# OllieBoyne/sslap

Hardware: AMD Instinct MI355X
Metric: Medges/s (bid-phase CSR nnz/s) + solve ms, N=200k d=0.1% sparse LAP (higher is better)
Workload: dtype f64

## Files before the change

### sslap_amd/csrc/host_base.hpp

```cpp
#pragma once

namespace {

thread_local std::string g_err;

int fail(int code, const char *fmt, ...) {
    char buf[512];
    va_list ap;
    va_start(ap, fmt);
    vsnprintf(buf, sizeof(buf), fmt, ap);
    va_end(ap);
    g_err = buf;
    return code;
}

#define HIP_TRY(expr)                                                                              \
    do {                                                                                           \
        hipError_t _e = (expr);                                                                    \
        if (_e != hipSuccess)                                                                      \
            return fail(MISSLAP_ERR_HIP, "%s failed: %s (%s:%d)", #expr, hipGetErrorString(_e), __FILE__, \
                        __LINE__);                                                                 \
    } while (0)

double now_ms() {
// ... 72 lines not shown
int block_alloc(void **p, size_t bytes, size_t *got);
void block_free(int device, void *p, size_t bytes);
}

namespace {
struct BatchFiber;
}
struct misslap_solver {
    BatchFiber *batch = nullptr;
    int abi = MISSLAP_ABI_VERSION;
    int n_cus = 256;
    double lines_safe_eps = 0.0;
    bool lines_dropped = false;
    double max_abs = 0.0;
    double pmax0 = 0.0;
    float eps_start_opt = 0.f;
    bool untouched = true;
    bool dense = false;
    int64_t dense_cols = 0;
    int device = 0;
    hipStream_t stream = nullptr;
    bool own_stream = false;
    int64_t nnz = 0;
    int n_rows = 0, n_cols = 0;
    int maximize = 0;
    bool f32 = true;
    int2 *edges32 = nullptr;
    int *col = nullptr;
    double *val64 = nullptr;
    int *row_ptr = nullptr;
    double *price = nullptr;
    float *price32 = nullptr;
    int *pmax_bits = nullptr;
    float cmax32 = 0.f;
    float *price32_buf = nullptr;
    PriceRec *rec = nullptr;
    int2 *cand = nullptr;
    double *cand64 = nullptr;
    int *p2o = nullptr, *o2p = nullptr, *U = nullptr;
    unsigned long long *bid_key = nullptr;
    int *bid_obj = nullptr;
    int4 *bid_rec = nullptr;
    unsigned long long *best_key = nullptr;
    int *best_pos = nullptr;
    int *cnt = nullptr, *hole_list = nullptr, *mover_list = nullptr;
    int *need_list = nullptr;
    Ctl *ctl = nullptr;
    double *contrib = nullptr;
    int *nmatch = nullptr;
    FinSlot *fin_slots = nullptr;
    int fin_slots_n = 0;
    unsigned long long *launch_edges = nullptr;
    int launch_edges_cap = 0;
    unsigned *tiled = nullptr;
    int tiled_fmt = 0;
    int *seg4 = nullptr;
    int *tcol = nullptr;
    int *ovf_ptr = nullptr;
    int4 *ovf_q = nullptr;
    int ovf_cap = 0;
    double2 *part_vw = nullptr;
    int *part_g = nullptr;
    unsigned long long *wg_stats = nullptr;
    int wg_stats_slots = 0;
    int take_edges_n = 0;
    unsigned long long *take_edges_out = nullptr;
    int *split_cnt = nullptr;
    int n_tiled = 0;
    int tile_cols = 0;
    long long tile_L = 0;
    int T = 0;
    bool tiled_ok = false;
    int tiled_min_K = 0;
    int tiled_shape = 0;
    std::vector<Blk> blocks;
    Ctl *h_ctl = nullptr;
    Ctl *h_stat = nullptr;
    volatile unsigned long long *live = nullptr;
    unsigned long long *live_dev = nullptr;
    unsigned ticket = 0;
    bool live_valid = false;
    bool live_off = false;
    bool live_every_round = false;
    unsigned slot_ticket[2] = {0, 0};
    bool slot_live[2] = {false, false};
    hipEvent_t stat_ev[2] = {nullptr, nullptr};
    float eps = 0, target_eps = 0, theta = 0, start_eps = 0;
    int nreductions = 0;
    bool finished = false;
    int64_t max_iter = 0;
    int thr = -1;
    bool round_small = false;
    bool round_fused = true;
    bool round_done = false;
    int cand_build_max_K = 0x7fffffff;
    int tail_round_budget = kLongRowTailBudget;
    int tail_launch_rounds = 1 << 22;
    int max_row_len = 0;
    long long avg_row_len = 0;
    bool lines_live() const { return cand != nullptr && !lines_dropped && (avg_row_len <= kCandRowMax || long_rows); }
    bool long_rows_later = false;
    long long tail_rounds_host = 0;
    long long tail_nits0 = -1;
    bool long_rows = false;
    bool long_rows0 = false, long_rows_later0 = false;
    bool line_maintenance = true;
    int cand_refresh_min = kDefaultCandRefresh;
    bool round_ordered = false;
    int apply_bidders_ratio = 2;
    bool profile_all = false;
    int rounds_per_sync = kDefaultRoundsPerSync;
    bool rounds_per_sync_auto = true;
    int rank = 0, world = 1;
    long long sharded_rounds = 0;
    int phases_run = 0, phases_with_lines = 0;
    int shard_min_K = 0;
    bool profile = false;
    int K_ub = 0;
    bool K_exact = false;
    bool walk_rev_next = false;
    bool ece_flag_clear = false;
    int ctl_fresh = 0;
    bool phase_fresh = true;
    std::vector<ProfRec> prof;
    size_t prof_used = 0;
    int launch_idx = 0;
    double setup_ms = 0, solve_ms = 0;
};
```

### sslap_amd/csrc/host_rounds.hpp

```cpp
#pragma once

namespace {
void begin_phase(misslap_solver *h) {
    if (h->cand != nullptr && !h->lines_dropped && (double)h->eps < h->lines_safe_eps) h->lines_dropped = true;
    h->phases_run += 1;
    h->phases_with_lines += h->lines_live() ? 1 : 0;
}

RoundArgs round_args(misslap_solver *h) {
    RoundArgs a;
    a.ctl = h->ctl;
    a.row_ptr = h->row_ptr;
    a.price = h->price;
    a.rec = h->rec;
    a.p2o = h->p2o;
    a.o2p = h->o2p;
    a.U = h->U;
    a.bid_key = h->bid_key;
    a.bid_obj = h->bid_obj;
    a.bid_rec = h->bid_rec;
    a.best_key = h->best_key;
    a.best_pos = h->best_pos;
    a.cnt = h->cnt;
    a.hole_list = h->hole_list;
// ... 17 lines not shown
    a.cand_build_max_K = h->cand_build_max_K;
    a.cand_build_min_K = (h->thr > 0 && h->line_maintenance) ? kRoundSmallMax : 0;
    a.cand_refresh_min = h->cand_refresh_min;
    a.price32 = nullptr;
    a.pmax_bits = h->pmax_bits;
    a.cmax = h->cmax32;
    return a;
}

int blocks_for(long long items, int per_block) {
    long long b = (items + per_block - 1) / per_block;
    if (b < 1) b = 1;
    if (b > kMaxGridBlocks) b = kMaxGridBlocks;
    return (int)b;
}

ProfRec *prof_next(misslap_solver *h, int kind) {
    if (h->prof_used == h->prof.size()) {
        ProfRec r{};
        if (hipEventCreate(&r.start) != hipSuccess || hipEventCreate(&r.stop) != hipSuccess) return nullptr;
        h->prof.push_back(r);
    }
    ProfRec *r = &h->prof[h->prof_used++];
    r->kind = kind;
    r->fullscan = 0;
    r->launch_idx = -1;
    return r;
}

void count_tail_rounds(misslap_solver *h) {
    if (h->tail_nits0 < 0) return;
    h->tail_rounds_host += h->h_ctl->nits - h->tail_nits0;
    h->tail_nits0 = -1;
}

int read_ctl(misslap_solver *h) {
    if (h->ctl_fresh == 2) {
        if (h->h_ctl->err)
            return fail(MISSLAP_ERR_STATE, "device-side invariant violated (error bits 0x%x)", h->h_ctl->err);
        return MISSLAP_OK;
    }
    HIP_TRY(stream_memcpy(h, h->h_ctl, h->ctl, sizeof(Ctl), hipMemcpyDeviceToHost));
    HIP_TRY(stream_sync(h));
    h->ctl_fresh = 2;
    h->K_ub = h->h_ctl->K;
    h->K_exact = true;
    count_tail_rounds(h);
    if (h->h_ctl->err)
        return fail(MISSLAP_ERR_STATE, "device-side invariant violated (error bits 0x%x)", h->h_ctl->err);
    return MISSLAP_OK;
}

bool live_poll(misslap_solver *h, unsigned want, bool exact, int *K, int *err, long long *nits) {
    volatile unsigned long long *w = h->live;
    double t_end = now_ms() + 20000.0;
    for (unsigned spins = 0;; ++spins) {
        const unsigned long long a = w[0], b = w[1], c = w[2], d = w[3];
        const unsigned t = (unsigned)(a >> 32);
        if ((unsigned)(b >> 32) == t && (unsigned)(c >> 32) == t && (unsigned)(d >> 32) == t && w[0] == a &&
            (exact ? t == want : (int)(t - want) >= 0)) {
            *K = (int)(unsigned)(a & 0xffffffffull);
            *err = (int)(unsigned)(b & 0xffffffffull);
            *nits = (long long)((c & 0xffffffffull) | ((d & 0xffffffffull) << 32));
            return true;
        }
        if (h->batch) {
            batch_yield(h, BatchFiber::kPolling);
            if (h->batch->at < h->batch->pending.size()) t_end = now_ms() + 20000.0;
            else if ((spins & 255) == 255 && now_ms() > t_end) return false;
        } else if (spins < 4000) {
            __builtin_ia32_pause();
        } else {
            std::this_thread::yield();
            if ((spins & 1023) == 0 && now_ms() > t_end) return false;
        }
    }
}
void ensure_posted(misslap_solver *h) {
    if (h->live_valid || h->live_off) return;
    launch<k_post_status>(h, dim3(1), h->ctl, h->live_dev, ++h->ticket);
    h->live_valid = true;
}
int read_status(misslap_solver *h) {
    if (h->ctl_fresh == 2 || h->live_off) return read_ctl(h);
    if (h->ctl_fresh == 1) {
        if (h->h_ctl->err) return fail(MISSLAP_ERR_STATE, "device-side invariant violated (error bits 0x%x)", h->h_ctl->err);
        return MISSLAP_OK;
    }
    ensure_posted(h);
    int K = 0, err = 0;
    long long nits = 0;
    if (!live_poll(h, h->ticket, true, &K, &err, &nits)) {
        h->live_off = true;
        return read_ctl(h);
    }
    h->h_ctl->K = K;
    h->h_ctl->nits = nits;
    h->h_ctl->err = err;
    h->K_ub = K;
    h->K_exact = true;
    count_tail_rounds(h);
    if (err) return fail(MISSLAP_ERR_STATE, "device-side invariant violated (error bits 0x%x)", err);
    return MISSLAP_OK;
}

int status_enqueue(misslap_solver *h, int slot) {
    h->slot_live[slot] = !h->live_off;
    if (h->slot_live[slot]) {
        ensure_posted(h);
        h->slot_ticket[slot] = h->ticket;
        return MISSLAP_OK;
    }
    h->ctl_fresh = false;
    if (h->batch) return fail(MISSLAP_ERR_STATE, "a batched solve needs the live status words");
    HIP_TRY(hipMemcpyAsync(&h->h_stat[slot], h->ctl, sizeof(Ctl), hipMemcpyDeviceToHost, h->stream));
    HIP_TRY(hipEventRecord(h->stat_ev[slot], h->stream));
    return MISSLAP_OK;
}
int status_wait(misslap_solver *h, int slot) {
    if (h->slot_live[slot]) {
        int K = 0, err = 0;
        long long nits = 0;
        if (live_poll(h, h->slot_ticket[slot], false, &K, &err, &nits)) {
            h->h_stat[slot].K = K;
            h->h_stat[slot].nits = nits;
            h->h_stat[slot].err = err;
            h->K_ub = K;
            h->K_exact = false;
            if (err) return fail(MISSLAP_ERR_STATE, "device-side invariant violated (error bits 0x%x)", err);
            return MISSLAP_OK;
        }
        h->live_off = true;
        int rc = read_ctl(h);
        h->h_stat[slot] = *h->h_ctl;
        h->K_exact = false;
        return rc;
    }
    HIP_TRY(hipEventSynchronize(h->stat_ev[slot]));
    const Ctl &c = h->h_stat[slot];
    h->K_ub = c.K;
    h->K_exact = false;
    if (c.err) return fail(MISSLAP_ERR_STATE, "device-side invariant violated (error bits 0x%x)", c.err);
    return MISSLAP_OK;
}

bool walk_backwards(misslap_solver *h, const int *shp) {
    const bool can = MISSLAP_TILED_KEYCOL_ON && h->tiled_fmt <= 1 && shp[7] == 1 &&
                     (h->tiled_shape == 0 || h->tiled_shape == 8 || h->tiled_shape == 9);
    if (h->phase_fresh) h->walk_rev_next = false;
    const bool rev = can && h->walk_rev_next;
    h->walk_rev_next = !h->walk_rev_next;
    return rev;
}

int launch_bid_tiled(misslap_solver *h) {
    h->ctl_fresh = false;
    RoundArgs a = round_args(h);
    const bool sharded = h->world > 1 && h->K_exact && h->K_ub >= h->shard_min_K;
    const long long share = sharded ? ((long long)h->K_ub + h->world - 1) / h->world : h->K_ub;
    const int *shp = kTiledShapes[h->tiled_shape];
    const int groups = (shp[0] - 64 * shp[5]) / shp[6];
    const int per_wg_max = groups * shp[1];
    const int cs = shp[7];
    long long grid = (share + per_wg_max - 1) / per_wg_max;
    const long long resident = h->n_cus / cs;
    const long long spread = std::min<long long>(resident, (share + groups - 1) / groups);
    if (grid < spread) grid = spread;
    grid *= cs;
    TiledArgs ta{h->tiled, h->tcol, h->seg4, h->T, h->tiled_min_K, h->n_tiled,
                 nullptr, nullptr, h->ovf_ptr, h->ovf_q, h->ovf_cap, h->part_vw, h->part_g, h->n_rows, h->split_cnt, FinalOut{}};
    h->round_ordered = !h->phase_fresh;
    if (h->round_ordered) {
        int *pos_of = h->nmatch, *order_person = h->hole_list, *order_pos = h->mover_list, *sums = h->cnt;
        const int nchunks = (h->n_rows + kScanChunk - 1) / kScanChunk;
        launch<k_order_prepare>(h, dim3(std::max(nchunks, blocks_for(h->K_ub, k_order_prepare::kBlock))), h->ctl, h->U, pos_of, h->p2o,
                                h->n_rows, nchunks, sums, h->thr, h->tiled_min_K);
        launch<k_order_scatter>(h, dim3(nchunks), h->ctl, h->p2o, h->n_rows, sums, pos_of, order_person, order_pos, h->thr, h->tiled_min_K);
        ta.order_person = order_person;
        ta.order_pos = order_pos;
    }
    if (grid > h->wg_stats_slots) return fail(MISSLAP_ERR_STATE, "scan grid %lld exceeds the statistics slots (%d)", grid, h->wg_stats_slots);
    ProfRec *pr = nullptr;
    if (h->profile) {
        if (h->launch_idx >= h->launch_edges_cap)
            return fail(MISSLAP_ERR_STATE, "profile buffer exhausted (%d bid launches)", h->launch_idx);
        pr = prof_next(h, 2);
        if (!pr) return fail(MISSLAP_ERR_HIP, "hipEventCreate failed");
        pr->fullscan = h->phase_fresh;
        pr->launch_idx = a.launch_idx = h->launch_idx++;
    }
    const size_t lds = tiled_lds_bytes(shp[4]);
    const dim3 g((unsigned)grid);
    if (walk_backwards(h, shp)) {
        const int key = h->tiled_fmt * 100 + shp[6];
        switch (key) {
#define X(FMT, GL) \
    case FMT * 100 + GL: launch_alone(h, pr, MISSLAP_BID_KERNEL_REV(GL, FMT), g, dim3(1024), lds, a, ta); break;
            X(0, 4) X(0, 8) X(0, 16) X(1, 4) X(1, 8) X(1, 16)
#undef X
            default: return fail(MISSLAP_ERR_STATE, "no backward instance for format %d with %d lanes per person", h->tiled_fmt, shp[6]);
        }
    } else if (h->tiled_fmt == 0) {
        switch (h->tiled_shape) {
#define X(I, TH, R, B, D, TC, LD, GL, CS) \
    case I: launch_alone(h, pr, k_bid_tiled<TH, R, B, D, TC, LD, 0, GL, CS>, g, dim3(TH), lds, a, ta); break;
            MISSLAP_FOR_TILED_SHAPES(X)
#undef X
            default: return fail(MISSLAP_ERR_STATE, "bad tiled shape");
        }
    } else {
        const int key = h->tiled_fmt * 100 + shp[6];
        switch (key) {
#define X(FMT, GL) \
    case FMT * 100 + GL: launch_alone(h, pr, MISSLAP_BID_KERNEL_FMT(GL, FMT), g, dim3(1024), lds, a, ta); break;
            MISSLAP_FOR_FMT_LANES(X)
#undef X
            default: return fail(MISSLAP_ERR_STATE, "no full-scan instance for format %d with %d lanes per person", h->tiled_fmt, shp[6]);
        }
    }
    if (pr) {
        h->take_edges_n = (int)grid;
        h->take_edges_out = h->launch_edges + 2 * (size_t)pr->launch_idx;
    }
    HIP_TRY(hipGetLastError());
    return MISSLAP_OK;
}

bool use_round_small(const misslap_solver *h) {
    return h->K_ub <= kRoundSmallMax && (h->world == 1 || h->K_ub < h->shard_min_K);
}

int launch_bid(misslap_solver *h) {
    h->ctl_fresh = false;
    h->untouched = false;
    h->round_small = use_round_small(h) && !(h->tiled_ok && h->K_ub >= h->tiled_min_K);
    if (h->tiled_ok && h->K_ub >= h->tiled_min_K) {
        int rc = launch_bid_tiled(h);
        if (rc) return rc;
        if (h->K_exact) {
            h->phase_fresh = false;
            h->K_exact = false;
            return MISSLAP_OK;
        }
    }
    h->K_exact = false;
    RoundArgs a = round_args(h);
    const long long share = h->K_ub;
    const bool fused = h->round_small && h->round_fused;
    const int grid = blocks_for(share, (fused ? 1024 : kBidBlock) / kWave);
    ProfRec *pr = nullptr;
    const bool fullscan = h->phase_fresh && !(h->tiled_ok && h->K_ub >= h->tiled_min_K);
    if (!(h->profile && (h->profile_all || fullscan))) a.launch_edges = nullptr;
    if (h->profile && (h->profile_all || fullscan)) {
        if (h->launch_idx >= h->launch_edges_cap)
            return fail(MISSLAP_ERR_STATE, "profile buffer exhausted (%d bid launches)", h->launch_idx);
        pr = prof_next(h, 0);
        if (!pr) return fail(MISSLAP_ERR_HIP, "hipEventCreate failed");
        pr->fullscan = fullscan;
        pr->launch_idx = a.launch_idx = h->launch_idx++;
    }
    const EdgesF32 e32{h->edges32};
    const EdgesF64 e64{h->col, h->val64};
    const dim3 g(grid);
    if (fused) {
        a.live = (h->live_off || !h->live_every_round) ? nullptr : h->live_dev;
        a.ticket = ++h->ticket;
        h->live_valid = a.live != nullptr;
    }
    const int variant = !h->lines_live() ? 0 : h->K_ub > h->cand_build_max_K ? 1 : 2;
    if (h->price32 && !h->round_small && variant != 2 && (long long)h->K_ub * 8 >= h->n_rows) {
        HIP_TRY(stream_memset(h, h->pmax_bits, 0, sizeof(int)));
        launch<k_price_mirror>(h, dim3(std::min(blocks_for(h->n_cols, k_price_mirror::kBlock * 4), h->n_cus)), h->ctl, h->price, h->price32,
                               h->n_cols, h->pmax_bits, h->thr, a.gather_max_K);
        a.price32 = h->price32;
    }
    const auto bid = [&](auto ed) {
        using E = decltype(ed);
        if (fused) launch_timed<k_round_fused<E>>(h, pr, g, a, ed);
        else if (h->round_small) launch_timed<k_bid<E, RecSource, 2>>(h, pr, g, a, ed);
        else if (variant == 0) launch_timed<k_bid<E, PriceSource, 0>>(h, pr, g, a, ed);
        else if (variant == 1) launch_timed<k_bid<E, PriceSource, 1>>(h, pr, g, a, ed);
        else launch_timed<k_bid<E, PriceSource, 2>>(h, pr, g, a, ed);
    };
    if (h->f32) bid(e32);
    else bid(e64);
    if (pr && !h->round_small) {
        h->take_edges_n = std::max(h->take_edges_n, grid);
        h->take_edges_out = h->launch_edges + 2 * (size_t)pr->launch_idx;
    } else if (pr) {
        hipLaunchKernelGGL(k_take_launch_edges, dim3(1), dim3(1024), 0, h->stream, h->wg_stats, grid, h->launch_edges + 2 * (size_t)pr->launch_idx);
    }
    HIP_TRY(hipGetLastError());
    h->phase_fresh = false;
    h->round_done = fused;
    return MISSLAP_OK;
}

int launch_tiebreak(misslap_solver *h) {
    h->ctl_fresh = false;
    if (h->round_small) return MISSLAP_OK;
    RoundArgs a = round_args(h);
    const long long share = h->K_ub;
    launch<k_tiebreak>(h, dim3(blocks_for(share, k_tiebreak::kBlock)), a, h->round_ordered ? h->mover_list : nullptr, h->tiled_min_K,
                       h->take_edges_n, h->take_edges_out);
    h->take_edges_n = 0;
    h->take_edges_out = nullptr;
    HIP_TRY(hipGetLastError());
    return MISSLAP_OK;
}

int launch_apply(misslap_solver *h) {
    h->ctl_fresh = false;
    if (h->round_small && h->round_done) {
        h->round_small = h->round_done = false;
        h->K_exact = false;
        return MISSLAP_OK;
    }
    RoundArgs a = round_args(h);
    a.live = (h->live_off || (h->round_small && !h->live_every_round)) ? nullptr : h->live_dev;
    a.ticket = ++h->ticket;
    h->live_valid = a.live != nullptr;
    if (h->round_small) {
        h->round_small = false;
        h->K_exact = false;
        launch<k_round_small>(h, dim3(1), a);
        HIP_TRY(hipGetLastError());
        return MISSLAP_OK;
    }
    h->K_exact = false;
    h->round_ordered = false;
    if ((h->world == 1 || h->K_ub < h->shard_min_K) && (long long)h->K_ub * h->apply_bidders_ratio <= h->n_cols)
        launch<k_apply_bidders>(h, dim3(blocks_for(h->K_ub, k_apply_bidders::kBlock)), a);
    else
        launch<k_apply>(h, dim3(blocks_for(h->n_cols, k_apply::kBlock)), a);
    if (h->K_ub <= kCompactSmallMax) {
        launch<k_compact_small>(h, dim3(1), a);
    } else {
        const int cb = blocks_for(h->K_ub, kChunk);
        launch<k_compact_count>(h, dim3(cb), a);
        launch<k_compact_scatter>(h, dim3(cb), a);
        launch<k_compact_fill>(h, dim3(blocks_for(h->K_ub, k_compact_fill::kBlock)), a);
    }
    HIP_TRY(hipGetLastError());
    return MISSLAP_OK;
}

int launch_tail(misslap_solver *h) {
    if (h->thr <= 0) return MISSLAP_OK;
// ... 169 lines not shown
```

### sslap_amd/csrc/kernels_round.hpp

```cpp
#pragma once
#include "device_common.hpp"

namespace misslap {

struct RoundArgs {
    Ctl *ctl;
    const int *row_ptr;
    double *price;
    PriceRec *rec;
    int *p2o;
    int *o2p;
    int *U;
    unsigned long long *bid_key;
    int *bid_obj;
    int4 *bid_rec;
    unsigned long long *best_key;
    int *best_pos;
    int *cnt;
    int *hole_list;
    int *mover_list;
    unsigned long long *launch_edges;
    int n_rows, n_cols;
    int thr;
    int rank, world;
// ... 43 lines not shown

constexpr int kBidBlock = 256;
template <class Src>
struct SrcOf;
template <>
struct SrcOf<PriceSource> {
    static constexpr bool kOwners = false;
    static __device__ __forceinline__ PriceSource make(const RoundArgs &a) { return PriceSource{a.price}; }
};
template <>
struct SrcOf<RecSource> {
    static constexpr bool kOwners = true;
    static __device__ __forceinline__ RecSource make(const RoundArgs &a) { return RecSource{a.rec}; }
};
struct BidTally {
    unsigned long long edges = 0, hit_edges = 0;
    int nb = 0, nh = 0, err = 0;
};
__device__ __forceinline__ void handover_store(unsigned long long *p, unsigned long long v) {
    __hip_atomic_store(p, v, __ATOMIC_RELAXED, __HIP_MEMORY_SCOPE_AGENT);
}
__device__ __forceinline__ unsigned long long handover_load(const unsigned long long *p) {
    return __hip_atomic_load(p, __ATOMIC_RELAXED, __HIP_MEMORY_SCOPE_AGENT);
}

template <class E, class Src, int kLines, bool kHandOver>
__device__ __forceinline__ void bid_positions(const RoundArgs &a, const E &ed, int lo, int hi, int first, int stride,
                                              int i_first, BidTally &tl) {
    const int lane = threadIdx.x & 63;
    const double eps = (double)a.eps;
    const Src src = SrcOf<Src>::make(a);
    double hint = 0.0;
    const bool lines = kLines > 0 && E::kCand && a.cand != nullptr;
    for (int n = lo + first; n < hi; n += stride) {
        const int i = n == first ? i_first : a.U[n];
        const int s = a.row_ptr[i], e = a.row_ptr[i + 1];
        CandBid b[2];
        b[0].hit = false;
        if (lines) {
            typename E::Slot sl = LineIO<typename E::Slot>::load(a.cand, a.cand64,
                                                                 (size_t)i * kCandLanes + (lane & (kCandLanes - 1)));
            int alive[2];
            cand_eval2(sl, true, false, src, eps, b, tl.err, NoEarly(), NoStamp(), alive);
            if (kLines == 2 && alive[0] < a.cand_refresh_min) b[0].hit = false;
        }
        if (!b[0].hit) {
            if (kLines == 2) {
                CandBuildArgs ba;
                const typename E::Raw none[4] = {};
                wave_bid_full<E, Src, false, false>(ed, src, s, e, none, eps, b[0], ba, tl.err);
                if (lines && ba.want && hi > a.cand_build_min_K) cand_build(a.cand, a.cand64, i, ba, eps, hint);
            } else if (!SrcOf<Src>::kOwners && a.price32 != nullptr) {
                const float two_delta = 0x1p-21f * (a.cmax + __int_as_float(*a.pmax_bits));
                wave_bid_filter(ed, a.price, a.price32, two_delta, s, e, eps, b[0], tl.err);
            } else {
                wave_bid_lean(ed, src, s, e, eps, b[0], tl.err);
            }
        } else {
            tl.nh += 1;
            tl.hit_edges += (unsigned long long)b[0].len;
        }
        if (lane == 0) {
            if (kHandOver) {
                handover_store(&a.bid_key[n], b[0].key);
                unsigned long long *r = reinterpret_cast<unsigned long long *>(&a.bid_rec[n]);
                handover_store(r, (unsigned long long)(unsigned)b[0].obj | ((unsigned long long)(unsigned)b[0].prev << 32));
                handover_store(r + 1, (unsigned long long)(unsigned)i | ((unsigned long long)(unsigned)s << 32));
            } else {
                a.bid_key[n] = b[0].key;
                if (SrcOf<Src>::kOwners) {
                    a.bid_rec[n] = make_int4(b[0].obj, b[0].prev, i, s);
                } else {
                    a.bid_obj[n] = b[0].obj;
                    atomicMax(&a.best_key[b[0].obj], b[0].key);
                }
            }
        }
        tl.edges += (unsigned long long)b[0].len;
        tl.nb += 1;
    }
}

template <int kWaves>
__device__ __forceinline__ void tally_flush(const RoundArgs &a, const BidTally &tl, int K) {
    const int wave = threadIdx.x >> 6, lane = threadIdx.x & 63;
    __shared__ unsigned long long s_edges[kWaves], s_hedges[kWaves];
    __shared__ int s_nb[kWaves], s_nh[kWaves];
    if (lane == 0) {
        s_edges[wave] = tl.edges;
        s_hedges[wave] = tl.hit_edges;
        s_nb[wave] = tl.nb;
        s_nh[wave] = tl.nh;
        if (tl.err) atomicOr(&a.ctl->err, tl.err);
    }
    __syncthreads();
    if (threadIdx.x == 0) {
        unsigned long long te = 0, the = 0;
        int tb = 0, th = 0;
        for (int w = 0; w < kWaves; ++w) {
            te += s_edges[w];
            the += s_hedges[w];
            tb += s_nb[w];
            th += s_nh[w];
        }
        if (tb) {
            unsigned long long *st = a.wg_stats + (size_t)kStatWords * blockIdx.x;
            st[kStatEdges] += te;
            st[kStatBids] += (unsigned long long)tb;
            if (a.world > 1 && K >= a.shard_min_K) st[kStatShardEdges] += te;
            if (a.launch_edges) {
                st[kStatLaunchEdges] += te;
                st[kStatLaunchHitEdges] += the;
            }
            if (th) {
                st[kStatHits] += (unsigned long long)th;
                st[kStatHitEdges] += the;
            }
        }
    }
}

template <class E, class Src, int kLines>
struct k_bid {
    MISSLAP_KERNEL(kBidBlock)
    static __device__ __forceinline__ void run(RoundArgs a, E ed) {
        static_assert(kLines == 2 || !SrcOf<Src>::kOwners, "the lean scan does not carry the owners k_round_small needs");
        const int wave = threadIdx.x >> 6;
        const int wpb = kBidBlock / kWave;
        const int first = blockIdx.x * wpb + wave;
        const Ctl *ctl = a.ctl;
        const CtlHead head(ctl);
        const int i_first = a.U[min(first, a.n_rows - 1)];
        if (!head.live(a.thr, i_first < -1)) return;
        if (a.gather_max_K > 0 && head.K >= a.gather_max_K) return;
        int lo, hi;
        shard_range(head.K, a.rank, a.world, a.shard_min_K, lo, hi);
        BidTally tl;
        bid_positions<E, Src, kLines, false>(a, ed, lo, hi, first, gridDim.x * wpb, i_first, tl);
        tally_flush<kBidBlock / kWave>(a, tl, head.K);
    }
};


struct k_price_mirror {
    MISSLAP_KERNEL(1024)
    static __device__ __forceinline__ void run(const Ctl *ctl, const double *price, float *price32, int n_cols, int *pmax_bits, int thr, int gather_max_K) {
        if (!round_live(ctl, thr) || (gather_max_K > 0 && ctl->K >= gather_max_K)) return;
        __shared__ int s_w[16];
        float m = 0.f;
        for (int j = blockIdx.x * blockDim.x + threadIdx.x; j < n_cols; j += gridDim.x * blockDim.x) {
            const float p = (float)price[j];
            price32[j] = p;
            m = __builtin_fmaxf(m, __builtin_fabsf(p));
        }
        int b = __float_as_int(m);
        for (int off = 32; off >= 1; off >>= 1) b = max(b, __shfl_xor(b, off));
        if ((threadIdx.x & 63) == 0) s_w[threadIdx.x >> 6] = b;
        __syncthreads();
        if (threadIdx.x == 0) {
            for (int w = 1; w < (int)blockDim.x / kWave; ++w) b = max(b, s_w[w]);
            if (b > 0) atomicMax(pmax_bits, b);
        }
    }
};


template <class E>
struct k_refresh_lines {
    MISSLAP_KERNEL(kBidBlock)
    static __device__ __forceinline__ void run(RoundArgs a, E ed, int min_alive, int long_max, int min_alive_long) {
        if (!E::kCand || a.cand == nullptr) return;
        const int wave = threadIdx.x >> 6, lane = threadIdx.x & 63;
        const int wpb = kBidBlock / kWave;
        const double eps = (double)a.eps;
        const PriceSource src{a.price};
        double hint = 0.0;
        int err = 0;
        for (int w = blockIdx.x * wpb + wave; 2 * w < a.n_rows; w += gridDim.x * wpb) {
            const int i0 = 2 * w, i1 = 2 * w + 1;
            const bool act1 = i1 < a.n_rows;
            const int ime = (lane < kCandLanes || !act1) ? i0 : i1;
            typename E::Slot sl = LineIO<typename E::Slot>::load(a.cand, a.cand64,
                                                                 (size_t)ime * kCandLanes + (lane & (kCandLanes - 1)));
            CandBid b[2];
            int alive[2];
            cand_eval2(sl, true, act1, src, eps, b, err, NoEarly(), NoStamp(), alive);
#pragma unroll
            for (int X = 0; X < 2; ++X) {
                if (X == 1 && !act1) continue;
                if (b[X].hit && alive[X] >= max(min_alive, min_alive_long)) continue;
                const int i = X ? i1 : i0;
                const int s = a.row_ptr[i], e = a.row_ptr[i + 1];
                if (e - s > kCandRowMax) {
                    if (long_max > 0 && e - s <= long_max && !(b[X].hit && alive[X] >= min_alive_long) && lane == 0)
                        a.need_list[atomicAdd(&a.ctl->n_need, 1)] = i;
                    continue;
                }
                if (b[X].hit && alive[X] >= min_alive) continue;
                CandBid full;
                CandBuildArgs ba;
                const typename E::Raw none[4] = {};
                wave_bid_full<E, PriceSource, false, false>(ed, src, s, e, none, eps, full, ba, err);
// ... 432 lines not shown
#pragma unroll
        for (int q = 0; q < kQ; ++q) un[q] = a.U[min(q * 1024 + t, K - 1)];
        for (int base = 0; base < K; base += kQ * 1024, par ^= 1) {
            int u[kQ];
            unsigned long long bl[kQ], bm[kQ];
            bool isl[kQ], ism[kQ];
#pragma unroll
            for (int q = 0; q < kQ; ++q) u[q] = un[q];
#pragma unroll
            for (int q = 0; q < kQ; ++q) {
                const int n = base + kQ * 1024 + q * 1024 + t;
                un[q] = a.U[min(n, K - 1)];
            }
#pragma unroll
            for (int q = 0; q < kQ; ++q) {
                const int n = base + q * 1024 + t;
                isl[q] = (n < Kn) & (u[q] == -1);
                ism[q] = (n >= Kn) & (n < K) & (u[q] != -1);
                bl[q] = __ballot(isl[q]);
                bm[q] = __ballot(ism[q]);
                if (lane == 0) {
                    s_w[par][0][q][wave] = __popcll(bl[q]);
                    s_w[par][1][q][wave] = __popcll(bm[q]);
                }
            }
            asm volatile("s_waitcnt lgkmcnt(0)\n\ts_barrier" ::: "memory");
            const int wave_s = __builtin_amdgcn_readfirstlane(wave);
#pragma unroll
            for (int q = 0; q < kQ; ++q) {
                const int n = base + q * 1024 + t;
                const int cx = lane < 16 ? s_w[par][0][q][lane & 15] : 0, cy = lane < 16 ? s_w[par][1][q][lane & 15] : 0;
                int x = cx, y = cy;
                x += __builtin_amdgcn_update_dpp(0, x, 0x111, 0xF, 0xF, true);
                y += __builtin_amdgcn_update_dpp(0, y, 0x111, 0xF, 0xF, true);
                x += __builtin_amdgcn_update_dpp(0, x, 0x112, 0xF, 0xF, true);
                y += __builtin_amdgcn_update_dpp(0, y, 0x112, 0xF, 0xF, true);
                x += __builtin_amdgcn_update_dpp(0, x, 0x114, 0xF, 0xF, true);
                y += __builtin_amdgcn_update_dpp(0, y, 0x114, 0xF, 0xF, true);
                x += __builtin_amdgcn_update_dpp(0, x, 0x118, 0xF, 0xF, true);
                y += __builtin_amdgcn_update_dpp(0, y, 0x118, 0xF, 0xF, true);
                const int wl = __builtin_amdgcn_readlane(x - cx, wave_s), wm = __builtin_amdgcn_readlane(y - cy, wave_s);
                const int tl = __builtin_amdgcn_readlane(x, 15), tm = __builtin_amdgcn_readlane(y, 15);
                if (isl[q]) a.hole_list[run_l + wl + __popcll(bl[q] & lanemask_lt())] = n;
                if (ism[q]) {
                    a.mover_list[run_m + wm + __popcll(bm[q] & lanemask_lt())] = u[q];
                    a.U[n] = -1;
                }
                run_l += tl;
                run_m += tm;
            }
        }
        __syncthreads();
        const int nl = run_l;
        for (int k = t; k < nl; k += 1024) a.U[a.hole_list[k]] = a.mover_list[k];
    }
    if (t == 0) {
        const long long nits = ctl->nits + 1;
        ctl->K = Kn;
        ctl->nholes = 0;
        ctl->nleft = 0;
        ctl->nits = nits;
        ctl->grid_rounds += 1;
        post_live_status(a.live, a.ticket, Kn, err_seen, nits);
    }
}

struct k_compact_small {
    MISSLAP_KERNEL(1024)
    static __device__ __forceinline__ void run(RoundArgs a) {
        Ctl *ctl = a.ctl;
        const CtlHead head(ctl);
        if (!head.live(a.thr, false)) {
            if (threadIdx.x == 0) post_live_status(a.live, a.ticket, head.K, head.err, head.nits);
            return;
        }
        compact_small_body(a, ctl, head.K, ctl->nholes, head.err);
    }
};


constexpr int kRoundSmallMax = 2048;
constexpr int kRoundSmallSlots = kRoundSmallMax / 1024;
constexpr int kRoundSmallHash = 2 * kRoundSmallMax;
__device__ __forceinline__ void round_small_body(const RoundArgs &a, Ctl *ctl, const CtlHead &head,
                                                 const int4 (&br)[kRoundSmallSlots],
                                                 const unsigned long long (&key)[kRoundSmallSlots]) {
    const int t = threadIdx.x, lane = t & 63, wave = t >> 6;
    const int K = head.K;
    __shared__ int s_cnt[16], s_wl[16], s_wm[16];
    __shared__ int s_hole[kRoundSmallMax], s_mover[kRoundSmallMax];
    __shared__ int hObj[kRoundSmallHash], hPos[kRoundSmallHash];
    __shared__ unsigned long long hKey[kRoundSmallHash];
    for (int h = t; h < kRoundSmallHash; h += 1024) {
        hObj[h] = -1;
        hKey[h] = 0ull;
        hPos[h] = kPosNone;
    }
    int obj[kRoundSmallSlots], who[kRoundSmallSlots], prev[kRoundSmallSlots], rstart[kRoundSmallSlots];
    int hs[kRoundSmallSlots];
#pragma unroll
    for (int q = 0; q < kRoundSmallSlots; ++q) {
        obj[q] = br[q].x;
        prev[q] = br[q].y;
        who[q] = br[q].z;
        rstart[q] = br[q].w;
    }
    __syncthreads();
#pragma unroll
    for (int q = 0; q < kRoundSmallSlots; ++q) {
        hs[q] = 0;
        if (q * 1024 + t < K) {
            int h = (int)(((unsigned)obj[q] * 2654435761u) >> 16) & (kRoundSmallHash - 1);
            for (;;) {
                const int old = atomicCAS(&hObj[h], -1, obj[q]);
                if (old == -1 || old == obj[q]) break;
                h = (h + 1) & (kRoundSmallHash - 1);
            }
            hs[q] = h;
            atomicMax(&hKey[h], key[q]);
        }
    }
    __syncthreads();
#pragma unroll
    for (int q = 0; q < kRoundSmallSlots; ++q)
        if (q * 1024 + t < K && hKey[hs[q]] == key[q]) atomicMin(&hPos[hs[q]], q * 1024 + t);
    __syncthreads();
    int bpos[kRoundSmallSlots];
#pragma unroll
    for (int q = 0; q < kRoundSmallSlots; ++q) bpos[q] = hPos[hs[q]];
    int holes = 0;
    int u[kRoundSmallSlots];
#pragma unroll
    for (int q = 0; q < kRoundSmallSlots; ++q) {
        const int n = q * 1024 + t, j = obj[q];
        u[q] = who[q];
        if (n < K && bpos[q] == n) {
            const int i = who[q];
            PriceRec r;
            r.price = key_to_bid(key[q]);
            r.owner = i;
            r.ostart = rstart[q];
            a.rec[j] = r;
            a.price[j] = r.price;
            if (prev[q] != -1) a.p2o[prev[q]] = -1;
            u[q] = prev[q];
            holes += prev[q] == -1;
            a.p2o[i] = j;
            a.o2p[j] = i;
        }
    }
    for (int off = 32; off >= 1; off >>= 1) holes += __shfl_xor(holes, off);
    if (lane == 0) s_cnt[wave] = holes;
    __syncthreads();
    int nholes = 0;
    for (int w = 0; w < 16; ++w) nholes += s_cnt[w];
    const int Kn = K - nholes;
    int cl = 0, cm = 0;
    unsigned filled = 0;
#pragma unroll
    for (int q = 0; q < kRoundSmallSlots; ++q) {
        const int n = q * 1024 + t;
        if (q * 1024 >= K) break;
        const bool isl = (n < Kn) && (u[q] == -1);
        const bool ism = (n >= Kn) && (n < K) && (u[q] != -1);
        const unsigned long long bl = __ballot(isl), bm = __ballot(ism);
        __syncthreads();
        if (lane == 0) {
            s_wl[wave] = __popcll(bl);
            s_wm[wave] = __popcll(bm);
        }
        __syncthreads();
        const int cx = lane < 16 ? s_wl[lane & 15] : 0, cy = lane < 16 ? s_wm[lane & 15] : 0;
        int x = cx, y = cy;
        x += __builtin_amdgcn_update_dpp(0, x, 0x111, 0xF, 0xF, true);
        y += __builtin_amdgcn_update_dpp(0, y, 0x111, 0xF, 0xF, true);
        x += __builtin_amdgcn_update_dpp(0, x, 0x112, 0xF, 0xF, true);
        y += __builtin_amdgcn_update_dpp(0, y, 0x112, 0xF, 0xF, true);
        x += __builtin_amdgcn_update_dpp(0, x, 0x114, 0xF, 0xF, true);
        y += __builtin_amdgcn_update_dpp(0, y, 0x114, 0xF, 0xF, true);
        x += __builtin_amdgcn_update_dpp(0, x, 0x118, 0xF, 0xF, true);
        y += __builtin_amdgcn_update_dpp(0, y, 0x118, 0xF, 0xF, true);
        const int wave_s = __builtin_amdgcn_readfirstlane(wave);
        const int wl = __builtin_amdgcn_readlane(x - cx, wave_s), wm = __builtin_amdgcn_readlane(y - cy, wave_s);
        const int tl = __builtin_amdgcn_readlane(x, 15), tm = __builtin_amdgcn_readlane(y, 15);
        if (ism) {
            s_mover[cm + wm + __popcll(bm & lanemask_lt())] = u[q];
            u[q] = -1;
        }
        if (isl) {
            s_hole[cl + wl + __popcll(bl & lanemask_lt())] = n;
            filled |= 1u << q;
        }
        cl += tl;
        cm += tm;
    }
    __syncthreads();
#pragma unroll
    for (int q = 0; q < kRoundSmallSlots; ++q) {
        const int n = q * 1024 + t;
        if (n < K && !((filled >> q) & 1u)) a.U[n] = u[q];
    }
    for (int k = t; k < cl; k += 1024) a.U[s_hole[k]] = s_mover[k];
    if (t == 0) {
        ctl->K = Kn;
        ctl->nholes = 0;
        ctl->nleft = 0;
        ctl->nits = head.nits + 1;
        ctl->grid_rounds += 1;
        post_live_status(a.live, a.ticket, Kn, head.err, head.nits + 1);
    }
}

struct k_round_small {
    MISSLAP_KERNEL(1024)
    static __device__ __forceinline__ void run(RoundArgs a) {
        const int t = threadIdx.x;
        Ctl *ctl = a.ctl;
        const CtlHead head(ctl);
        int4 br[kRoundSmallSlots];
        unsigned long long key[kRoundSmallSlots];
        bool never = false;
#pragma unroll
        for (int q = 0; q < kRoundSmallSlots; ++q) {
            br[q] = a.bid_rec[q * 1024 + t];
            key[q] = a.bid_key[min(q * 1024 + t, a.n_rows - 1)];
            never |= (br[q].x < 0) | (key[q] == ~0ull);
        }
        if (!head.live(a.thr, never)) {
            if (t == 0) post_live_status(a.live, a.ticket, head.K, head.err, head.nits);
            return;
        }
        round_small_body(a, ctl, head, br, key);
    }
};


template <class E>
struct k_round_fused {
    MISSLAP_KERNEL(1024)
    static __device__ __forceinline__ void run(RoundArgs a, E ed) {
        const int t = threadIdx.x, wave = t >> 6;
        constexpr int wpb = 1024 / kWave;
        const int first = blockIdx.x * wpb + wave;
        Ctl *ctl = a.ctl;
        const CtlHead head(ctl);
        const int i_first = a.U[min(first, a.n_rows - 1)];
        asm volatile("" ::"v"(i_first));
        if (!head.live(a.thr, false)) {
            if (blockIdx.x == 0 && t == 0) post_live_status(a.live, a.ticket, head.K, head.err, head.nits);
            return;
        }
        BidTally tl;
        bid_positions<E, RecSource, 2, true>(a, ed, 0, head.K, first, gridDim.x * wpb, i_first, tl);
        tally_flush<wpb>(a, tl, head.K);
        __shared__ int s_arrived;
        asm volatile("s_waitcnt vmcnt(0)" ::: "memory");
        __syncthreads();
        if (t == 0) s_arrived = __hip_atomic_fetch_add(&ctl->arrive, 1, __ATOMIC_RELAXED, __HIP_MEMORY_SCOPE_AGENT);
        __syncthreads();
        if (s_arrived != (int)gridDim.x - 1) return;
        if (t == 0) __hip_atomic_store(&ctl->arrive, 0, __ATOMIC_RELAXED, __HIP_MEMORY_SCOPE_AGENT);
        int4 br[kRoundSmallSlots];
        unsigned long long key[kRoundSmallSlots];
#pragma unroll
        for (int q = 0; q < kRoundSmallSlots; ++q) {
            const int n = min(q * 1024 + t, a.n_rows - 1);
            const unsigned long long *r = reinterpret_cast<const unsigned long long *>(&a.bid_rec[q * 1024 + t]);
            const unsigned long long r0 = handover_load(r), r1 = handover_load(r + 1);
            br[q] = make_int4((int)(unsigned)(r0 & 0xffffffffull), (int)(unsigned)(r0 >> 32), (int)(unsigned)(r1 & 0xffffffffull),
                              (int)(unsigned)(r1 >> 32));
            key[q] = handover_load(&a.bid_key[n]);
        }
        round_small_body(a, ctl, head, br, key);
    }
};


struct k_post_status {
    MISSLAP_KERNEL_BOUND(1, 1024)
    static __device__ __forceinline__ void run(const Ctl *ctl, unsigned long long *live, unsigned ticket) {
        post_live_status(live, ticket, ctl->K, ctl->err, ctl->nits);
    }
};

struct k_post_ece {
    MISSLAP_KERNEL_BOUND(1, 1024)
    static __device__ __forceinline__ void run(const Ctl *ctl, unsigned long long *live, unsigned ticket) {
        post_live_status(live, ticket, ctl->K, ctl->err, ctl->nits);
        __hip_atomic_store(&live[4], ((unsigned long long)ticket << 32) | (unsigned)ctl->ece_fail, __ATOMIC_RELAXED, __HIP_MEMORY_SCOPE_SYSTEM);
    }
};


struct k_reset_phase {
    MISSLAP_KERNEL(256)
    static __device__ __forceinline__ void run(Ctl *ctl, int *p2o, int *o2p, PriceRec *rec, int *U, int n_rows, int n_cols) {
        const int stride = gridDim.x * blockDim.x;
        const int t = blockIdx.x * blockDim.x + threadIdx.x;
        for (int i = t; i < n_rows; i += stride) {
            p2o[i] = -1;
            U[i] = i;
        }
        for (int j = t; j < n_cols; j += stride) {
            o2p[j] = -1;
            rec[j].owner = -1;
        }
        if (t == 0) {
            ctl->K = n_rows;
            ctl->nholes = 0;
            ctl->nleft = 0;
            ctl->arrive = 0;
            ctl->ece_fail = 0;
        }
    }
};


}
```

Baseline: 5389.

## Defer fused-round tally stores off the critical arrive path, specialize small-K resolve

```diff
diff --git a/sslap_amd/csrc/host_base.hpp b/sslap_amd/csrc/host_base.hpp
--- a/sslap_amd/csrc/host_base.hpp
+++ b/sslap_amd/csrc/host_base.hpp
@@ -178,6 +178,7 @@
     bool live_valid = false;
     bool live_off = false;
     bool live_every_round = false;
+    int fused_since_post = 0;
     unsigned slot_ticket[2] = {0, 0};
     bool slot_live[2] = {false, false};
     hipEvent_t stat_ev[2] = {nullptr, nullptr};
diff --git a/sslap_amd/csrc/host_rounds.hpp b/sslap_amd/csrc/host_rounds.hpp
--- a/sslap_amd/csrc/host_rounds.hpp
+++ b/sslap_amd/csrc/host_rounds.hpp
@@ -123,6 +123,7 @@
     h->live_valid = true;
 }
 int read_status(misslap_solver *h) {
+    h->fused_since_post = 0;
     if (h->ctl_fresh == 2 || h->live_off) return read_ctl(h);
     if (h->ctl_fresh == 1) {
         if (h->h_ctl->err) return fail(MISSLAP_ERR_STATE, "device-side invariant violated (error bits 0x%x)", h->h_ctl->err);
@@ -146,6 +147,7 @@
 }
 
 int status_enqueue(misslap_solver *h, int slot) {
+    h->fused_since_post = 0;
     h->slot_live[slot] = !h->live_off;
     if (h->slot_live[slot]) {
         ensure_posted(h);
@@ -304,7 +306,9 @@
     const EdgesF64 e64{h->col, h->val64};
     const dim3 g(grid);
     if (fused) {
-        a.live = (h->live_off || !h->live_every_round) ? nullptr : h->live_dev;
+        h->fused_since_post += 1;
+        const bool closes_batch = h->rounds_per_sync_auto && h->fused_since_post == kRoundsPerSyncLive;
+        a.live = (h->live_off || !(h->live_every_round || closes_batch)) ? nullptr : h->live_dev;
         a.ticket = ++h->ticket;
         h->live_valid = a.live != nullptr;
     }
diff --git a/sslap_amd/csrc/kernels_round.hpp b/sslap_amd/csrc/kernels_round.hpp
--- a/sslap_amd/csrc/kernels_round.hpp
+++ b/sslap_amd/csrc/kernels_round.hpp
@@ -149,42 +149,55 @@
 }
 
 template <int kWaves>
+struct TallyLds {
+    unsigned long long edges[kWaves], hedges[kWaves];
+    int nb[kWaves], nh[kWaves];
+};
+template <int kWaves>
+__device__ __forceinline__ void tally_publish(const RoundArgs &a, const BidTally &tl, TallyLds<kWaves> &s) {
+    const int wave = threadIdx.x >> 6, lane = threadIdx.x & 63;
+    if (lane == 0) {
+        s.edges[wave] = tl.edges;
+        s.hedges[wave] = tl.hit_edges;
+        s.nb[wave] = tl.nb;
+        s.nh[wave] = tl.nh;
+        if (tl.err) atomicOr(&a.ctl->err, tl.err);
+    }
+}
+template <int kWaves, bool kNoWait>
+__device__ __forceinline__ void tally_add(const RoundArgs &a, const TallyLds<kWaves> &s, int K) {
+    unsigned long long te = 0, the = 0;
+    int tb = 0, th = 0;
+    for (int w = 0; w < kWaves; ++w) {
+        te += s.edges[w];
+        the += s.hedges[w];
+        tb += s.nb[w];
+        th += s.nh[w];
+    }
+    if (!tb) return;
+    unsigned long long *st = a.wg_stats + (size_t)kStatWords * blockIdx.x;
+    const auto add = [&](int k, unsigned long long v) {
+        if (kNoWait) __hip_atomic_fetch_add(&st[k], v, __ATOMIC_RELAXED, __HIP_MEMORY_SCOPE_WORKGROUP);
+        else st[k] += v;
+    };
+    add(kStatEdges, te);
+    add(kStatBids, (unsigned long long)tb);
+    if (a.world > 1 && K >= a.shard_min_K) add(kStatShardEdges, te);
+    if (a.launch_edges) {
+        add(kStatLaunchEdges, te);
+        add(kStatLaunchHitEdges, the);
+    }
+    if (th) {
+        add(kStatHits, (unsigned long long)th);
+        add(kStatHitEdges, the);
+    }
+}
+template <int kWaves>
 __device__ __forceinline__ void tally_flush(const RoundArgs &a, const BidTally &tl, int K) {
-    const int wave = threadIdx.x >> 6, lane = threadIdx.x & 63;
-    __shared__ unsigned long long s_edges[kWaves], s_hedges[kWaves];
-    __shared__ int s_nb[kWaves], s_nh[kWaves];
-    if (lane == 0) {
-        s_edges[wave] = tl.edges;
-        s_hedges[wave] = tl.hit_edges;
-        s_nb[wave] = tl.nb;
-        s_nh[wave] = tl.nh;
-        if (tl.err) atomicOr(&a.ctl->err, tl.err);
-    }
+    __shared__ TallyLds<kWaves> s;
+    tally_publish(a, tl, s);
     __syncthreads();
-    if (threadIdx.x == 0) {
-        unsigned long long te = 0, the = 0;
-        int tb = 0, th = 0;
-        for (int w = 0; w < kWaves; ++w) {
-            te += s_edges[w];
-            the += s_hedges[w];
-            tb += s_nb[w];
-            th += s_nh[w];
-        }
-        if (tb) {
-            unsigned long long *st = a.wg_stats + (size_t)kStatWords * blockIdx.x;
-            st[kStatEdges] += te;
-            st[kStatBids] += (unsigned long long)tb;
-            if (a.world > 1 && K >= a.shard_min_K) st[kStatShardEdges] += te;
-            if (a.launch_edges) {
-                st[kStatLaunchEdges] += te;
-                st[kStatLaunchHitEdges] += the;
-            }
-            if (th) {
-                st[kStatHits] += (unsigned long long)th;
-                st[kStatHitEdges] += the;
-            }
-        }
-    }
+    if (threadIdx.x == 0) tally_add<kWaves, false>(a, s, K);
 }
 
 template <class E, class Src, int kLines>
@@ -783,24 +796,30 @@
 constexpr int kRoundSmallMax = 2048;
 constexpr int kRoundSmallSlots = kRoundSmallMax / 1024;
 constexpr int kRoundSmallHash = 2 * kRoundSmallMax;
-__device__ __forceinline__ void round_small_body(const RoundArgs &a, Ctl *ctl, const CtlHead &head,
-                                                 const int4 (&br)[kRoundSmallSlots],
-                                                 const unsigned long long (&key)[kRoundSmallSlots]) {
+struct RoundSmallLds {
+    unsigned long long hKey[kRoundSmallHash];
+    int hObj[kRoundSmallHash], hPos[kRoundSmallHash];
+    int hole[kRoundSmallMax], mover[kRoundSmallMax];
+    int cnt[16], wl[16], wm[16];
+};
+template <int kSlots>
+__device__ __forceinline__ void round_small_body(const RoundArgs &a, Ctl *ctl, const CtlHead &head, RoundSmallLds &L,
+                                                 const int4 (&br)[kSlots], const unsigned long long (&key)[kSlots]) {
     const int t = threadIdx.x, lane = t & 63, wave = t >> 6;
     const int K = head.K;
-    __shared__ int s_cnt[16], s_wl[16], s_wm[16];
-    __shared__ int s_hole[kRoundSmallMax], s_mover[kRoundSmallMax];
-    __shared__ int hObj[kRoundSmallHash], hPos[kRoundSmallHash];
-    __shared__ unsigned long long hKey[kRoundSmallHash];
+    int (&s_cnt)[16] = L.cnt, (&s_wl)[16] = L.wl, (&s_wm)[16] = L.wm;
+    int (&s_hole)[kRoundSmallMax] = L.hole, (&s_mover)[kRoundSmallMax] = L.mover;
+    int (&hObj)[kRoundSmallHash] = L.hObj, (&hPos)[kRoundSmallHash] = L.hPos;
+    unsigned long long (&hKey)[kRoundSmallHash] = L.hKey;
     for (int h = t; h < kRoundSmallHash; h += 1024) {
         hObj[h] = -1;
         hKey[h] = 0ull;
         hPos[h] = kPosNone;
     }
-    int obj[kRoundSmallSlots], who[kRoundSmallSlots], prev[kRoundSmallSlots], rstart[kRoundSmallSlots];
-    int hs[kRoundSmallSlots];
-#pragma unroll
-    for (int q = 0; q < kRoundSmallSlots; ++q) {
+    int obj[kSlots], who[kSlots], prev[kSlots], rstart[kSlots];
+    int hs[kSlots];
+#pragma unroll
+    for (int q = 0; q < kSlots; ++q) {
         obj[q] = br[q].x;
         prev[q] = br[q].y;
         who[q] = br[q].z;
@@ -808,7 +827,7 @@
     }
     __syncthreads();
 #pragma unroll
-    for (int q = 0; q < kRoundSmallSlots; ++q) {
+    for (int q = 0; q < kSlots; ++q) {
         hs[q] = 0;
         if (q * 1024 + t < K) {
             int h = (int)(((unsigned)obj[q] * 2654435761u) >> 16) & (kRoundSmallHash - 1);
@@ -823,16 +842,16 @@
     }
     __syncthreads();
 #pragma unroll
-    for (int q = 0; q < kRoundSmallSlots; ++q)
+    for (int q = 0; q < kSlots; ++q)
         if (q * 1024 + t < K && hKey[hs[q]] == key[q]) atomicMin(&hPos[hs[q]], q * 1024 + t);
     __syncthreads();
-    int bpos[kRoundSmallSlots];
-#pragma unroll
-    for (int q = 0; q < kRoundSmallSlots; ++q) bpos[q] = hPos[hs[q]];
+    int bpos[kSlots];
+#pragma unroll
+    for (int q = 0; q < kSlots; ++q) bpos[q] = hPos[hs[q]];
     int holes = 0;
-    int u[kRoundSmallSlots];
-#pragma unroll
-    for (int q = 0; q < kRoundSmallSlots; ++q) {
+    int u[kSlots];
+#pragma unroll
+    for (int q = 0; q < kSlots; ++q) {
         const int n = q * 1024 + t, j = obj[q];
         u[q] = who[q];
         if (n < K && bpos[q] == n) {
@@ -859,7 +878,7 @@
     int cl = 0, cm = 0;
     unsigned filled = 0;
 #pragma unroll
-    for (int q = 0; q < kRoundSmallSlots; ++q) {
+    for (int q = 0; q < kSlots; ++q) {
         const int n = q * 1024 + t;
         if (q * 1024 >= K) break;
         const bool isl = (n < Kn) && (u[q] == -1);
@@ -897,7 +916,7 @@
     }
     __syncthreads();
 #pragma unroll
-    for (int q = 0; q < kRoundSmallSlots; ++q) {
+    for (int q = 0; q < kSlots; ++q) {
         const int n = q * 1024 + t;
         if (n < K && !((filled >> q) & 1u)) a.U[n] = u[q];
     }
@@ -931,7 +950,8 @@
             if (t == 0) post_live_status(a.live, a.ticket, head.K, head.err, head.nits);
             return;
         }
-        round_small_body(a, ctl, head, br, key);
+        __shared__ RoundSmallLds L;
+        round_small_body<kRoundSmallSlots>(a, ctl, head, L, br, key);
     }
 };
 
@@ -953,26 +973,43 @@
         }
         BidTally tl;
         bid_positions<E, RecSource, 2, true>(a, ed, 0, head.K, first, gridDim.x * wpb, i_first, tl);
-        tally_flush<wpb>(a, tl, head.K);
+        __shared__ TallyLds<wpb> s_tally;
+        __shared__ RoundSmallLds L;
         __shared__ int s_arrived;
+        tally_publish(a, tl, s_tally);
         asm volatile("s_waitcnt vmcnt(0)" ::: "memory");
         __syncthreads();
         if (t == 0) s_arrived = __hip_atomic_fetch_add(&ctl->arrive, 1, __ATOMIC_RELAXED, __HIP_MEMORY_SCOPE_AGENT);
         __syncthreads();
-        if (s_arrived != (int)gridDim.x - 1) return;
+        if (s_arrived != (int)gridDim.x - 1) {
+            if (t == 0) tally_add<wpb, true>(a, s_tally, head.K);
+            return;
+        }
         if (t == 0) __hip_atomic_store(&ctl->arrive, 0, __ATOMIC_RELAXED, __HIP_MEMORY_SCOPE_AGENT);
-        int4 br[kRoundSmallSlots];
-        unsigned long long key[kRoundSmallSlots];
-#pragma unroll
-        for (int q = 0; q < kRoundSmallSlots; ++q) {
+        if (head.K <= 1024) resolve<1>(a, ctl, head, s_tally, L);
+        else resolve<kRoundSmallSlots>(a, ctl, head, s_tally, L);
+    }
+    template <int kSlots>
+    static __device__ __forceinline__ void resolve(const RoundArgs &a, Ctl *ctl, const CtlHead &head,
+                                                   const TallyLds<1024 / kWave> &s_tally, RoundSmallLds &L) {
+        const int t = threadIdx.x;
+        int4 br[kSlots];
+        unsigned long long key[kSlots];
+        unsigned long long r0[kSlots], r1[kSlots];
+#pragma unroll
+        for (int q = 0; q < kSlots; ++q) {
             const int n = min(q * 1024 + t, a.n_rows - 1);
             const unsigned long long *r = reinterpret_cast<const unsigned long long *>(&a.bid_rec[q * 1024 + t]);
-            const unsigned long long r0 = handover_load(r), r1 = handover_load(r + 1);
-            br[q] = make_int4((int)(unsigned)(r0 & 0xffffffffull), (int)(unsigned)(r0 >> 32), (int)(unsigned)(r1 & 0xffffffffull),
-                              (int)(unsigned)(r1 >> 32));
+            r0[q] = handover_load(r);
+            r1[q] = handover_load(r + 1);
             key[q] = handover_load(&a.bid_key[n]);
         }
-        round_small_body(a, ctl, head, br, key);
+        if (t == 0) tally_add<1024 / kWave, true>(a, s_tally, head.K);
+#pragma unroll
+        for (int q = 0; q < kSlots; ++q)
+            br[q] = make_int4((int)(unsigned)(r0[q] & 0xffffffffull), (int)(unsigned)(r0[q] >> 32), (int)(unsigned)(r1[q] & 0xffffffffull),
+                              (int)(unsigned)(r1[q] >> 32));
+        round_small_body<kSlots>(a, ctl, head, L, br, key);
     }
 };
 
```

Result: no change. 5408, median of 6 (+0.4%).
